# unlikeghost/DeepLearning-MPI

Measured on AMD Instinct MI355X. Metric: images/sec (whole node) ResNet-50 DDP bs=256/GPU, higher is better.
Workload: dtype bf16; 1 GPU; model=resnet50, global_batch=256, image=224, in_channels=3, per_gpu_batch=256, parallelism=dp1, backend=single, device=cuda, optimizer=SGD(momentum=0.9, wd=1e-5), hipgraph=False

## Files before the change

deeplearning_mpi_amd/csrc/binding/conv_fwd.cpp:

```cpp
#include <algorithm>
#include <cstdio>
#include <map>
#include <vector>

#include "common.h"

namespace dlmpi_ext {

using dlmpi::ConvArgs;
using dlmpi::ConvPhase;
using dlmpi::FinArgs;
using dlmpi::Stream1x1Args;
using dlmpi::make_fastdiv;

void apply_halo(ConvArgs& a, int N, int bm) {
  ConvPhase& p = a.ph[0];
  int th = 8, tw = 16, tiles_h = 1, tiles_w = 1;
  halo_geom(p.P, p.Q, bm, th, tw, tiles_h, tiles_w);
  a.halo = 1;
  a.th = th;
  a.tw = tw;
  a.tiles_h = tiles_h;
  a.tiles_w = tiles_w;
  a.fd_tw = make_fastdiv((uint32_t)tw);
// ... 282 lines not shown
      const bool c8 = pl.path == FwdPath::c8;
      check((c8 ? dlmpi_conv3x3_c8 : dlmpi_conv4x4_c16)(a.x, ldx, xoff, N, H, W, a.w, a.bias, a.y, ldy, yoff, a.stats,
                                                        pl.G, cur_stream()),
            c8 ? "conv2d_fwd (8-channel 3x3)" : "conv2d_fwd (stem 4x4 x 16 channels)");
      (c8 ? g_ran.c8 : g_ran.c16) = 1;
      break;
    }
    case FwdPath::head:
      check(dlmpi_head1x1(a.x, ldx, xoff, (int64_t)N * H * W, C, a.w, a.ldw, a.bias, a.y, ldy, yoff, a.kvalid,
                          o.y_f32 ? 1 : 0, nullptr, nullptr, cur_stream()),
            "conv2d_fwd (1x1 head)");
      g_ran.head = 1;
      return 0;
    case FwdPath::stream3x3: {
      dlmpi::Conv3StreamArgs c = conv3_args(x, N, H, W, ldx, xoff, w, 0, a.y, ldy, yoff, pl.th, pl.tw, pl.G);
      c.bias = a.bias;
      c.stats = a.stats;
      check(dlmpi_conv3x3_stream(&c, a.stats ? 0 : 1, cur_stream()), "conv2d_fwd (stream 3x3)");
      g_ran.conv3 = 1;
      break;
    }
    case FwdPath::stream1x1: {
      Stream1x1Args sa = fill_stream1x1(x, ldx, xoff, w, y, ldy, yoff, s.M(), C, K, a.bias, H, W, P, Q, pl.sbm,
                                        pl.sbn, pl.G);
      sa.stats = a.stats;
      sa.s2 = stride == 2 ? 1 : 0;
      check(dlmpi_conv1x1_stream(&sa, pl.sbm, pl.sbn, cur_stream()), "conv2d_fwd (stream 1x1)");
      g_ran.stream = 1;
      break;
    }
    case FwdPath::apply1x1:
      a.ntiles = ceil_div(K, bn);
      single_phase(a, P, Q, R, S, pad, bm);
      check(dlmpi_conv1x1_apply(&a, bm, cur_stream()), "conv2d_fwd (fused apply 1x1)");
      break;
    case FwdPath::pipe:
    case FwdPath::halo:
    case FwdPath::igemm:
      a.ntiles = ceil_div(K, bn);
      single_phase(a, P, Q, R, S, pad, bm);
      if (pl.path == FwdPath::halo) apply_halo(a, N, bm);
      g_ran.halo = pl.path == FwdPath::halo ? 1 : 0;
      if (!pl.pipe && (fin != nullptr || !a.stats) && s.free_tiles() && autotune(a, 0, bm, bn)) rows = a.ph[0].mtiles;
      if (fin != nullptr) need_rows(rows);
      if (g_sw.splitk > 0) a.splitk_req = g_sw.splitk;
      check(dlmpi_conv_igemm_ex(&a, bm, bn, pl.pipe, cur_stream()), "conv2d_fwd");
      break;
  }
  if (fin != nullptr) run_fin_after(*stats, rows, K, fin);
  return rows;
}

int conv2d_fwd_pro(const at::Tensor& x, int N, int H, int W, int C, int ldx, int xoff, const at::Tensor& w, int K, int R,
               int S, int stride, int pad, at::Tensor y, int ldy, int yoff, const c10::optional<at::Tensor>& bias,
               const c10::optional<at::Tensor>& res, int ldres, int resoff, const c10::optional<at::Tensor>& scale,
               const c10::optional<at::Tensor>& shift, bool relu, const c10::optional<at::Tensor>& stats, int bm_req,
               int kvalid, int bn_req, int pro, const c10::optional<at::Tensor>& pk0,
               const c10::optional<at::Tensor>& pk1, const c10::optional<at::Tensor>& pz, int ldpz, int pzoff) {
  return conv2d_fwd_impl(x, N, H, W, C, ldx, xoff, w, K, R, S, stride, pad, y, ldy, yoff, bias, res, ldres, resoff,
                         scale, shift, relu, stats, bm_req, kvalid, bn_req, pro, pk0, pk1, pz, ldpz, pzoff, nullptr);
}

int conv2d_fwd(const at::Tensor& x, int N, int H, int W, int C, int ldx, int xoff, const at::Tensor& w, int K, int R,
               int S, int stride, int pad, at::Tensor y, int ldy, int yoff, const c10::optional<at::Tensor>& bias,
               const c10::optional<at::Tensor>& res, int ldres, int resoff, const c10::optional<at::Tensor>& scale,
               const c10::optional<at::Tensor>& shift, bool relu, const c10::optional<at::Tensor>& stats, int bm_req,
               int kvalid, int bn_req) {
// ... 190 lines not shown
  check(dlmpi_conv_igemm(&a, t.bm, t.bn, cur_stream()), "convT2x2_fwd");
}

void register_conv_fwd(pybind11::module& m) {
  m.def("conv2d_fwd", &conv2d_fwd);
  m.def("conv2d_fwd_pro", &conv2d_fwd_pro);
  m.def("conv2d_fwd_bn", &conv2d_fwd_bn);
  m.def("conv2d_fwd_bn_apply", &conv2d_fwd_bn_apply);
  m.def("conv2d_fwd_mtiles", &conv2d_fwd_mtiles);
  m.def("conv2d_fwd_mtiles_pro", &conv2d_fwd_mtiles_pro);
  m.def("conv2d_fwd_plan", &conv2d_fwd_plan);
  m.def("conv_tune_tiles", [](int f32, int C, int K) {
    std::vector<std::pair<int, int>> v;
    for (const TuneCand& c : tune_candidates(f32, C, K, 0)) v.emplace_back(c.bm, c.bn);
    return v;
  });
  m.def("conv2d_fwd_bnbwd", &conv2d_fwd_bnbwd);
  m.def("convT2x2_fwd", &convT2x2_fwd);
  m.def("conv1x1_head_affine", &conv1x1_head_affine);
  m.def("conv3_pro_ok", &conv3_pro_ok);
  m.def("conv3x3_fwd_bn_apply", &conv3x3_fwd_bn_apply);
  m.def("clear_conv_plans", []() { g_conv_plans.clear(); });
  m.def("set_conv_stream", [](int mode) { dlmpi_set_conv_stream(mode); });
  m.def("set_conv3_stream", [](int mode) { dlmpi_set_conv3_stream(mode); });
  m.def("set_halo_pipe", [](int on) { dlmpi_set_halo_pipe(on); });
  m.def("set_dgs_blocks", [](int n) { dlmpi_set_dgs_blocks(n); });
  m.def("dgs_blocks", []() { return dlmpi_dgs_blocks(); });
  def_int(m, "set_conv_autotune", nullptr, &g_sw.autotune);
  def_int(m, "set_conv_halo", nullptr, &g_sw.halo);
  def_int(m, "set_halo_first", nullptr, &g_sw.halo_first);
  def_int(m, "set_conv_splitk", nullptr, &g_sw.splitk);
  def_int(m, "set_conv_pipe", nullptr, &g_sw.pipe);
  def_int(m, "set_conv_apply", nullptr, &g_sw.apply);
  def_int(m, "set_head1x1", "head1x1_on", &g_sw.head);
  def_int(m, "set_conv_c8", nullptr, &g_sw.c8);
  def_int(m, "set_conv_c16", nullptr, &g_sw.c16);
  def_int(m, "set_conv3_pro", nullptr, &g_sw.c3pro);
  def_int(m, "set_convT_stream", nullptr, &g_sw.convT_stream);
  def_int(m, nullptr, "conv_stream_last", &g_ran.stream);
  def_int(m, nullptr, "conv3_stream_last", &g_ran.conv3);
  def_int(m, nullptr, "conv_halo_last", &g_ran.halo);
  def_int(m, nullptr, "conv_c8_last", &g_ran.c8);
  def_int(m, nullptr, "conv_c16_last", &g_ran.c16);
  def_int(m, nullptr, "head1x1_last", &g_ran.head);
  def_int(m, nullptr, "convT_stream_last", &g_ran.convT_stream);
}

}
```

deeplearning_mpi_amd/csrc/binding/conv_plan.h:

```cpp
#pragma once
#include <cstdint>
#include <vector>

#include "../kernels/dlmpi_kernels.h"

namespace dlmpi_ext {

static inline int ceil_div(int64_t a, int64_t b) { return (int)((a + b - 1) / b); }

struct Switches {
  int pipe = -1;
  int pipe_dgrad = -1;
  int apply = -1;
  int halo = -1;
  int halo_first = 1;
  int splitk = 0;
  int autotune = -1;
  int head = 1;
  int c8 = 1;
  int c16 = 1;
  int c3pro = 1;
  int convT_stream = 1;
  int wgrad3 = -1;
  int wgrad3_blocks = 0;
  int wgrad_blocks = 0;
};
struct LastRan {
  int halo = 0;
  int stream = 0;
  int dgrad_stream = 0;
  int conv3 = 0;
  int head = 0;
  int c8 = 0;
  int c16 = 0;
  int convT_stream = 0;
  int wgrad3 = 0;
  int head_dgrad = 0;
};
extern Switches g_sw;
extern LastRan g_ran;
bool conv_autotune_on();

struct ConvShape {
  int N, H, W, C, K, R, S, stride, pad;
  int pro, f32;
  int bm_req, bn_req;
// ... 62 lines not shown
```

deeplearning_mpi_amd/csrc/kernels/conv_igemm.hip:

```cpp
#include <cstdlib>
#include <type_traits>

#include "common.h"

namespace dlmpi {

typedef __attribute__((address_space(3))) void lds_void;

__device__ __forceinline__ void glds16(const void* g, char* lds_wave_base) {
  __builtin_amdgcn_global_load_lds(g, (lds_void*)lds_wave_base, 16, 0, 0);
}

template <int BM, int BN, int NT, int WM>
struct EpiSmem {
  static constexpr int NP0 = BM < 128 ? 1 : (BM / 64 < WM / 16 ? BM / 64 : WM / 16);
  static constexpr int NP = (WM / 16) % NP0 == 0 ? NP0 : WM / 16;
  static constexpr int CS_LD = BN + 4;
  static constexpr int EPI = (BM / NP) * CS_LD * 4;
  static constexpr int RED = (NT / (BN / 8)) * 3 * BN * 4;
  static constexpr int bytes = EPI > RED ? EPI : RED;
};

template <int NT, int NF>
__device__ __forceinline__ bool splitk_combine(const ConvArgs& a, f32x4* acc, char* smem, int tid, int mt, int nt) {
  const int S = a.splitk;
  const int64_t tile = (int64_t)blockIdx.z * gridDim.x + (int64_t)mt * a.ntiles + nt;
  f32x4* slab = reinterpret_cast<f32x4*>(a.sk_slab) + (tile * S + blockIdx.y) * NF * NT + tid;
#pragma unroll
  for (int i = 0; i < NF; ++i) slab[(int64_t)i * NT] = acc[i];
  asm volatile("s_waitcnt vmcnt(0)" ::: "memory");
  __syncthreads();
  int* flag = reinterpret_cast<int*>(smem);
  if (tid == 0) {
    __builtin_amdgcn_fence(__ATOMIC_RELEASE, "agent");
    asm volatile("s_waitcnt vmcnt(0)" ::: "memory");
    flag[0] = __hip_atomic_fetch_add(a.sk_tk + tile, 1, __ATOMIC_RELAXED, __HIP_MEMORY_SCOPE_AGENT) == S - 1;
  }
  __syncthreads();
  if (!flag[0]) return false;
  if (tid == 0) {
    __builtin_amdgcn_fence(__ATOMIC_ACQUIRE, "agent");
    asm volatile("s_waitcnt vmcnt(0)" ::: "memory");
    __hip_atomic_store(a.sk_tk + tile, 0, __ATOMIC_RELAXED, __HIP_MEMORY_SCOPE_AGENT);
  }
  __syncthreads();
  const f32x4* base = reinterpret_cast<const f32x4*>(a.sk_slab) + tile * S * NF * NT + tid;
#pragma unroll
  for (int i = 0; i < NF; ++i) acc[i] = f32x4{0.f, 0.f, 0.f, 0.f};
  for (int sp = 0; sp < S; ++sp)
#pragma unroll
    for (int i = 0; i < NF; ++i) acc[i] += base[((int64_t)sp * NF + i) * NT];
  __syncthreads();
  return true;
}

template <int BM, int BN, int NT, int WGM, int WGN, typename T, bool HALO>
__device__ __forceinline__ void conv_epilogue(const ConvArgs& a, const ConvPhase& ph,
                                              f32x4 (&acc)[BM / WGM / 16][BN / WGN / 16], char* smem, int tid,
                                              int m0, int n0, int mt, int hn, int hh0, int hw0) {
  constexpr int WM = BM / WGM, WN = BN / WGN;
  constexpr int TM = WM / 16, TN = WN / 16;
  constexpr int NP = EpiSmem<BM, BN, NT, WM>::NP;
  constexpr int CS_LD = EpiSmem<BM, BN, NT, WM>::CS_LD;
  static_assert(WM % (16 * NP) == 0 || NP == 1, "epilogue pass must split every wave's rows evenly");
  const int lane = tid & 63;
  const int wid = __builtin_amdgcn_readfirstlane(tid >> 6);
  const int wm = wid / WGN, wn = wid % WGN;
  const int fr = lane & 15, fg = lane >> 4;
  const int PQ = ph.P * ph.Q;
  const int M = a.Nimg * PQ;
  float* Cs = reinterpret_cast<float*>(smem);

  constexpr int CG = BN / 8;
  constexpr int RG = NT / CG;
  const int cg = tid % CG, rg = tid / CG;
  const int c0 = n0 + cg * 8;
  const bool cvalid = c0 < a.Kout;
  float bias[8];
#pragma unroll
  for (int e = 0; e < 8; ++e) bias[e] = 0.f;
  if (cvalid && a.bias) {
#pragma unroll
    for (int e = 0; e < 8; ++e) bias[e] = a.bias[c0 + e];
  }
  float s1[8], s2[8], s3[8];
#pragma unroll
  for (int e = 0; e < 8; ++e) { s1[e] = 0.f; s2[e] = 0.f; s3[e] = 0.f; }
  const bool bwd = a.mask != nullptr || a.mscale != nullptr || a.mbits != nullptr;

  constexpr int HM = WM / NP, HT = TM / NP;
#pragma unroll
  for (int h = 0; h < NP; ++h) {
  if (h) __syncthreads();
#pragma unroll
  for (int mi = 0; mi < HT; ++mi)
#pragma unroll
    for (int ni = 0; ni < TN; ++ni)
#pragma unroll
      for (int r = 0; r < 4; ++r)
        Cs[(wm * HM + mi * 16 + fg * 4 + r) * CS_LD + wn * WN + ni * 16 + fr] = acc[h * HT + mi][ni][r];
  __syncthreads();
  constexpr int EPI_UNROLL = BM >= 256 ? 1 : 2;
#pragma unroll EPI_UNROLL
  for (int rr = rg; rr < BM / NP; rr += RG) {
    const int r = (rr / HM) * WM + h * HM + (rr % HM);
    const int m = m0 + r;
    int64_t pix;
    if constexpr (HALO) {
      const int pr = (int)fdiv((uint32_t)r, a.fd_tw), pc = r - pr * a.tw;
      const int oh = hh0 + pr, ow = hw0 + pc;
      if (r >= a.th * a.tw || oh >= ph.P || ow >= ph.Q || !cvalid) continue;
      pix = ((int64_t)hn * a.OH + oh * a.so + ph.oh0) * a.OW + ow * a.so + ph.ow0;
    } else {
      if (m >= M || !cvalid) continue;
    }
    float v[8];
    const f32x4 v0 = *reinterpret_cast<const f32x4*>(Cs + rr * CS_LD + cg * 8);
    const f32x4 v1 = *reinterpret_cast<const f32x4*>(Cs + rr * CS_LD + cg * 8 + 4);
#pragma unroll
    for (int e = 0; e < 4; ++e) { v[e] = v0[e] + bias[e]; v[e + 4] = v1[e] + bias[e + 4]; }
    if (a.stats && !bwd) {
#pragma unroll
      for (int e = 0; e < 8; ++e) {
        const float rv = stored<T>(v[e]);
        s1[e] += rv;
        s2[e] += rv * rv;
      }
    }
    if (a.scale) {
#pragma unroll
      for (int e = 0; e < 8; ++e) v[e] = v[e] * a.scale[c0 + e] + a.shift[c0 + e];
    }
    if constexpr (!HALO) {
      const uint32_t n_img = fdiv((uint32_t)m, ph.fdPQ);
      const uint32_t rem = (uint32_t)m - n_img * PQ;
      const uint32_t p = fdiv(rem, ph.fdQ);
      const uint32_t q = rem - p * ph.Q;
      pix = ((int64_t)n_img * a.OH + (int)p * a.so + ph.oh0) * a.OW + (int)q * a.so + ph.ow0;
    }
    if (a.res) {
      float rr8[8];
      load8(static_cast<const T*>(a.res) + pix * a.ldres + a.resoff + c0, rr8);
#pragma unroll
      for (int e = 0; e < 8; ++e) v[e] += rr8[e];
    }
    if (a.relu) {
#pragma unroll
      for (int e = 0; e < 8; ++e) v[e] = fmaxf(v[e], 0.f);
    }
    if (bwd) {
      float zz[8];
      if (a.z) load8(static_cast<const T*>(a.z) + pix * a.ldz + a.zoff + c0, zz);
      if (a.mbits) {
        const uint32_t b = a.mbits[pix * (a.Kout >> 3) + (c0 >> 3)];
#pragma unroll
        for (int e = 0; e < 8; ++e) v[e] = (b >> e) & 1u ? v[e] : 0.f;
      } else if (a.mask) {
        float yy[8];
        load8(static_cast<const T*>(a.mask) + pix * a.ldmask + a.maskoff + c0, yy);
#pragma unroll
        for (int e = 0; e < 8; ++e) v[e] = yy[e] > 0.f ? v[e] : 0.f;
      } else {
#pragma unroll
        for (int e = 0; e < 8; ++e) v[e] = zz[e] * a.mscale[c0 + e] + a.mshift[c0 + e] > 0.f ? v[e] : 0.f;
      }
      if (a.stats) {
#pragma unroll
        for (int e = 0; e < 8; ++e) {
          const float rv = stored<T>(v[e]);
          s1[e] += rv;
          s2[e] += rv * zz[e];
        }
        if (a.z2) {
          load8(static_cast<const T*>(a.z2) + pix * a.ldz2 + a.z2off + c0, zz);
#pragma unroll
          for (int e = 0; e < 8; ++e) s3[e] += stored<T>(v[e]) * zz[e];
        }
      }
    }
    if (a.vec_store) {
      if (a.out_f32) {
        float* yp = reinterpret_cast<float*>(a.y) + pix * a.ldy + a.yoff + c0;
        *reinterpret_cast<f32x4*>(yp) = f32x4{v[0], v[1], v[2], v[3]};
        *reinterpret_cast<f32x4*>(yp + 4) = f32x4{v[4], v[5], v[6], v[7]};
      } else {
        uint16_t* yp = reinterpret_cast<uint16_t*>(a.y) + pix * a.ldy + a.yoff + c0;
        *reinterpret_cast<u32x4*>(yp) = pack8(v);
      }
    } else {
#pragma unroll
      for (int e = 0; e < 8; ++e) {
        if (c0 + e >= a.kvalid) break;
        if (a.out_f32) reinterpret_cast<float*>(a.y)[pix * a.ldy + a.yoff + c0 + e] = v[e];
        else reinterpret_cast<uint16_t*>(a.y)[pix * a.ldy + a.yoff + c0 + e] = f2bf(v[e]);
      }
    }
  }
  }

  if (a.stats) {
    __syncthreads();
    float* red = reinterpret_cast<float*>(smem);
    const int ns = a.nstat;
#pragma unroll
    for (int e = 0; e < 8; ++e) {
      red[(rg * 3 + 0) * BN + cg * 8 + e] = s1[e];
      red[(rg * 3 + 1) * BN + cg * 8 + e] = s2[e];
      red[(rg * 3 + 2) * BN + cg * 8 + e] = s3[e];
    }
    __syncthreads();
    if (tid < BN && n0 + tid < a.Kout) {
      float t1 = 0.f, t2 = 0.f, t3 = 0.f;
      for (int g = 0; g < RG; ++g) {
// ... 703 lines not shown
      bf16x8 af[TM], bfr[TN];
#pragma unroll
      for (int ni = 0; ni < TN; ++ni)
        bfr[ni] = *reinterpret_cast<const bf16x8*>(smem + b_row0 + sl * B_BYTES + ni * 16 * 128 + ((ch ^ sw) << 4));
#pragma unroll
      for (int mi = 0; mi < TM; ++mi)
        af[mi] = *reinterpret_cast<const bf16x8*>(smem + (kk ? (a_addr[mi] ^ 64) : a_addr[mi]));
      if (kk == 0 && more && !chunk_end) {
        issue_b(sl ^ 1);
        asm volatile("" ::: "memory");
      }
#pragma unroll
      for (int mi = 0; mi < TM; ++mi)
#pragma unroll
        for (int ni = 0; ni < TN; ++ni)
          acc[mi][ni] = __builtin_amdgcn_mfma_f32_16x16x32_bf16(af[mi], bfr[ni], acc[mi][ni], 0, 0, 0);
    }
    if (chunk_end) {
      asm volatile("s_waitcnt lgkmcnt(0)" ::: "memory");
      __builtin_amdgcn_s_barrier();
      asm volatile("" ::: "memory");
      issue_halo();
      issue_b(sl ^ 1);
    }
  };
  for (int ks = 0; ks < nk; ks += 2) {
    step(ks, std::integral_constant<int, 0>{});
    if (ks + 1 < nk) step(ks + 1, std::integral_constant<int, 1>{});
  }
  __syncthreads();
  conv_epilogue<BM, BN, NT, WGM, WGN, uint16_t, true>(a, ph, acc, smem, tid, m0, n0, mt, hn, hh0, hw0);
}

template <int BM, int BN, int WGM, int WGN>
__global__ __launch_bounds__(512) __attribute__((amdgpu_waves_per_eu(BN <= 128 ? 4 : 2, 8)))
void conv1x1_apply_kernel(const ConvArgs a) {
  constexpr int NT = 512;
  static_assert(WGM * WGN == 8, "8 waves");
  constexpr int WM = BM / WGM, WN = BN / WGN, TM = WM / 16, TN = WN / 16;
  constexpr int A_BYTES = BM * 128, B_BYTES = BN * 128, SB = A_BYTES + B_BYTES;
  constexpr int MAXC = 4 * BN;
  constexpr int PRM_BYTES = 4 * MAXC * 4;
  constexpr int EPI_NEED = EpiSmem<BM, BN, NT, WM>::bytes;
  constexpr int SMEM = 2 * SB + PRM_BYTES > EPI_NEED ? 2 * SB + PRM_BYTES : EPI_NEED;
  constexpr int RP = NT / 8;
  constexpr int AL = BM / RP, BL = BN / RP;
  static_assert(AL >= 1 && BL >= 1, "tile shape");
  __shared__ __attribute__((aligned(16))) char smem[SMEM];

  const int tid = threadIdx.x, lane = tid & 63;
  const int wid = __builtin_amdgcn_readfirstlane(tid >> 6);
  const int wm = wid / WGN, wn = wid % WGN;
  const int lrow = tid >> 3, jc = tid & 7;
  const ConvPhase& ph = a.ph[0];
  const int M = a.Nimg * ph.P * ph.Q;
  const uint32_t mt = xcd_remap(blockIdx.x, (uint32_t)ph.mtiles);
  const int m0 = (int)mt * BM;
  const int C = a.C, nk = C / 64;
  const bool rbn = a.prscale != nullptr;

  float* prm = reinterpret_cast<float*>(smem + 2 * SB);
  for (int i = tid; i < C; i += NT) {
    prm[i] = a.pscale[i];
    prm[MAXC + i] = a.pshift[i];
    if (rbn) {
      prm[2 * MAXC + i] = a.prscale[i];
      prm[3 * MAXC + i] = a.prshift[i];
    }
  }

  const uint16_t* xb = static_cast<const uint16_t*>(a.x);
  const uint16_t* rb = static_cast<const uint16_t*>(a.pz);
  uint32_t zo[AL], ro[AL], yo[AL], bo[AL];
  uint32_t okm = 0;
#pragma unroll
  for (int i = 0; i < AL; ++i) {
    const int m = m0 + lrow + RP * i;
    if (m < M) okm |= 1u << i;
    const uint32_t mm = m < M ? (uint32_t)m : 0u;
    zo[i] = mm * (uint32_t)a.ldx + (uint32_t)a.xoff + 8 * jc;
    ro[i] = mm * (uint32_t)a.ldpz + (uint32_t)a.pzoff + 8 * jc;
    yo[i] = mm * (uint32_t)a.ldpy + (uint32_t)a.pyoff + 8 * jc;
    bo[i] = mm * (uint32_t)(C >> 3) + jc;
  }
  const uint16_t* wb = static_cast<const uint16_t*>(a.w) + (int64_t)lrow * a.ldw + 8 * jc;
  const int64_t wstep = (int64_t)RP * a.ldw;

  u32x4 zv[AL], rv[AL], wv[BL];
  auto load = [&](int k) {
    const int c = 64 * k;
#pragma unroll
    for (int i = 0; i < AL; ++i) {
      zv[i] = *reinterpret_cast<const u32x4*>(xb + zo[i] + c);
      rv[i] = *reinterpret_cast<const u32x4*>(rb + ro[i] + c);
    }
#pragma unroll
    for (int i = 0; i < BL; ++i) wv[i] = *reinterpret_cast<const u32x4*>(wb + i * wstep + c);
  };
  auto commit = [&](int k, int buf) {
    char* As = smem + buf * SB;
    char* Bs = As + A_BYTES;
    const int cc = 64 * k + 8 * jc;
    const f32x4 s0 = *reinterpret_cast<const f32x4*>(prm + cc), s1 = *reinterpret_cast<const f32x4*>(prm + cc + 4);
    const f32x4 h0 = *reinterpret_cast<const f32x4*>(prm + MAXC + cc);
    const f32x4 h1 = *reinterpret_cast<const f32x4*>(prm + MAXC + cc + 4);
#pragma unroll
    for (int i = 0; i < AL; ++i) {
      const int r = lrow + RP * i;
      u32x4 pk = u32x4{0u, 0u, 0u, 0u};
      if ((okm >> i) & 1) {
        float v[8], q[8];
        unpack8(zv[i], v);
        unpack8(rv[i], q);
#pragma unroll
        for (int e = 0; e < 4; ++e) {
          v[e] = __builtin_fmaf(v[e], s0[e], h0[e]);
          v[e + 4] = __builtin_fmaf(v[e + 4], s1[e], h1[e]);
        }
        if (rbn) {
          const f32x4 a0 = *reinterpret_cast<const f32x4*>(prm + 2 * MAXC + cc);
          const f32x4 a1 = *reinterpret_cast<const f32x4*>(prm + 2 * MAXC + cc + 4);
          const f32x4 b0 = *reinterpret_cast<const f32x4*>(prm + 3 * MAXC + cc);
          const f32x4 b1 = *reinterpret_cast<const f32x4*>(prm + 3 * MAXC + cc + 4);
#pragma unroll
          for (int e = 0; e < 4; ++e) {
            q[e] = __builtin_fmaf(q[e], a0[e], b0[e]);
            q[e + 4] = __builtin_fmaf(q[e + 4], a1[e], b1[e]);
          }
        }
#pragma unroll
        for (int e = 0; e < 8; ++e) v[e] = fmaxf(v[e] + q[e], 0.f);
        pk = pack8(v);
        *reinterpret_cast<u32x4*>(a.py + yo[i] + 64 * k) = pk;
        uint32_t b = 0;
#pragma unroll
        for (int t = 0; t < 4; ++t) {
          b |= (uint32_t)((pk[t] & 0xffffu) != 0u && !(pk[t] & 0x8000u)) << (2 * t);
          b |= (uint32_t)((pk[t] >> 16) != 0u && !(pk[t] & 0x80000000u)) << (2 * t + 1);
        }
        a.pmbits[bo[i] + 8 * k] = (uint8_t)b;
      }
      *reinterpret_cast<u32x4*>(As + r * 128 + ((jc ^ (r & 7)) << 4)) = pk;
    }
#pragma unroll
    for (int i = 0; i < BL; ++i) {
      const int r = lrow + RP * i;
      *reinterpret_cast<u32x4*>(Bs + r * 128 + ((jc ^ (r & 7)) << 4)) = wv[i];
    }
  };

  f32x4 acc[TM][TN];
#pragma unroll
  for (int mi = 0; mi < TM; ++mi)
#pragma unroll
    for (int ni = 0; ni < TN; ++ni) acc[mi][ni] = f32x4{0.f, 0.f, 0.f, 0.f};
  const int fr = lane & 15, fg = lane >> 4;

  load(0);
  __syncthreads();
  commit(0, 0);
  __syncthreads();
  for (int k = 0; k < nk; ++k) {
    if (k + 1 < nk) load(k + 1);
    const char* As = smem + (k & 1) * SB;
    const char* Bs = As + A_BYTES;
#pragma unroll
    for (int kk = 0; kk < 2; ++kk) {
      bf16x8 af[TM], bfr[TN];
      const int ch = kk * 4 + fg;
#pragma unroll
      for (int mi = 0; mi < TM; ++mi) {
        const int r = wm * WM + mi * 16 + fr;
        af[mi] = *reinterpret_cast<const bf16x8*>(As + r * 128 + ((ch ^ (r & 7)) << 4));
      }
#pragma unroll
      for (int ni = 0; ni < TN; ++ni) {
        const int r = wn * WN + ni * 16 + fr;
        bfr[ni] = *reinterpret_cast<const bf16x8*>(Bs + r * 128 + ((ch ^ (r & 7)) << 4));
      }
#pragma unroll
      for (int mi = 0; mi < TM; ++mi)
#pragma unroll
        for (int ni = 0; ni < TN; ++ni)
          acc[mi][ni] = __builtin_amdgcn_mfma_f32_16x16x32_bf16(af[mi], bfr[ni], acc[mi][ni], 0, 0, 0);
    }
    if (k + 1 < nk) commit(k + 1, (k + 1) & 1);
    __syncthreads();
  }
  conv_epilogue<BM, BN, NT, WGM, WGN, uint16_t, false>(a, ph, acc, smem, tid, m0, 0, (int)mt, 0, 0, 0);
}

}

using namespace dlmpi;

template <int BM, int BN>
static hipError_t launch_tile(const ConvArgs* a, dim3 grid, hipStream_t s) {
  if (a->pro == 3) {
    if constexpr (BM == 128 && BN == 64) hipLaunchKernelGGL((conv_igemm_kernel<BM, BN, false, 2, 3>), grid, dim3(256), 0, s, *a);
    else return hipErrorInvalidValue;
  } else if (a->C < 64) hipLaunchKernelGGL((conv_igemm_kernel<BM, BN, true, 2>), grid, dim3(256), 0, s, *a);
  else hipLaunchKernelGGL((conv_igemm_kernel<BM, BN, false, 2>), grid, dim3(256), 0, s, *a);
  return hipSuccess;
}

static int splitk_plan(int tiles, int nk) {
  if (tiles >= 256 || nk < 8) return 1;
  int S = (256 + tiles - 1) / tiles;
  S = S < nk / 4 ? S : nk / 4;
  S = S < 8 ? S : 8;
  return S < 2 ? 1 : S;
}

static hipError_t launch_f32(const ConvArgs* a, int bm, int bn, dim3 grid, hipStream_t s) {
  if (a->pro != 0) return hipErrorInvalidValue;
  const bool small = a->C < 32 || a->C % 32 != 0;
#define LAUNCH_F32(BM_, BN_)                                                                                   \
  do {                                                                                                       \
    if (small) hipLaunchKernelGGL((conv_igemm_kernel<BM_, BN_, true, 2, 0, float>), grid, dim3(256), 0, s, *a); \
    else hipLaunchKernelGGL((conv_igemm_kernel<BM_, BN_, false, 2, 0, float>), grid, dim3(256), 0, s, *a);     \
  } while (0)
  if (bm == 128 && bn == 128) LAUNCH_F32(128, 128);
  else if (bm == 128 && bn == 64) LAUNCH_F32(128, 64);
  else if (bm == 64 && bn == 128) LAUNCH_F32(64, 128);
  else if (bm == 64 && bn == 64) LAUNCH_F32(64, 64);
  else return hipErrorInvalidValue;
#undef LAUNCH_F32
  return hipGetLastError();
}

static hipError_t launch_pipe(const ConvArgs* a, int bm, int bn, int var, dim3 grid, hipStream_t s) {
  if (a->f32 || a->pro != 0 || a->C % 64 != 0 || a->C > kPipeMaxC || a->halo || grid.y != 1) return hipErrorInvalidValue;
  if (var != (bm == 128 ? 4 : 2)) return hipErrorInvalidValue;
  if (bm == 256 && bn == 256) hipLaunchKernelGGL((conv_pipe_kernel<256, 256, 2, 4, 2, 2>), grid, dim3(512), 0, s, *a);
  else if (bm == 224 && bn == 256) hipLaunchKernelGGL((conv_pipe_kernel<224, 256, 2, 4, 2, 2>), grid, dim3(512), 0, s, *a);
  else if (bm == 256 && bn == 128) hipLaunchKernelGGL((conv_pipe_kernel<256, 128, 4, 2, 3, 2>), grid, dim3(512), 0, s, *a);
  else if (bm == 128 && bn == 256) hipLaunchKernelGGL((conv_pipe_kernel<128, 256, 2, 4, 3, 4>), grid, dim3(512), 0, s, *a);
  else if (bm == 512 && bn == 64) hipLaunchKernelGGL((conv_pipe_kernel<512, 64, 8, 1, 2, 2>), grid, dim3(512), 0, s, *a);
  else return hipErrorInvalidValue;
  return hipGetLastError();
}

extern "C" int dlmpi_conv1x1_apply_ok(int C, int K) {
  return C % 64 == 0 && C <= 4 * K && (K == 64 || K == 128 || K == 256);
}

extern "C" hipError_t dlmpi_conv1x1_apply(const ConvArgs* a, int bm, hipStream_t s) {
  if (a->pro != 3 || a->f32 || a->halo || a->nphase != 1 || a->ntiles != 1 || !a->vec_store || a->res ||
      a->scale || a->relu || a->mask || a->mscale || a->mbits || a->z || a->splitk_req > 1 ||
      !dlmpi_conv1x1_apply_ok(a->C, a->Kout) || a->ph[0].Tr != 1 || a->ph[0].Ts != 1 || a->sa != 1 ||
      a->ph[0].mtiles != (a->Nimg * a->ph[0].P * a->ph[0].Q + bm - 1) / bm || a->ldw != a->C ||
      (int64_t)a->Nimg * a->H * a->W * (a->ldx > a->ldpz ? (a->ldx > a->ldpy ? a->ldx : a->ldpy)
                                                          : (a->ldpz > a->ldpy ? a->ldpz : a->ldpy)) >= (1ll << 31))
    return hipErrorInvalidValue;
  const dim3 grid((unsigned)a->ph[0].mtiles);
  if (grid.x == 0) return hipSuccess;
  if (bm == 128 && a->Kout == 64) hipLaunchKernelGGL((conv1x1_apply_kernel<128, 64, 8, 1>), grid, dim3(512), 0, s, *a);
  else if (bm == 128 && a->Kout == 128) hipLaunchKernelGGL((conv1x1_apply_kernel<128, 128, 4, 2>), grid, dim3(512), 0, s, *a);
  else if (bm == 128 && a->Kout == 256) hipLaunchKernelGGL((conv1x1_apply_kernel<128, 256, 2, 4>), grid, dim3(512), 0, s, *a);
  else return hipErrorInvalidValue;
  return hipGetLastError();
}

static int g_halo_pipe = 1;
extern "C" void dlmpi_set_halo_pipe(int on) { g_halo_pipe = on; }

extern "C" hipError_t dlmpi_conv_igemm_ex(const ConvArgs* a_in, int bm, int bn, int pipe, hipStream_t s) {
  int maxt = 0, tiles = 0, maxk = 0;
  for (int i = 0; i < a_in->nphase; ++i) {
    maxt = a_in->ph[i].mtiles > maxt ? a_in->ph[i].mtiles : maxt;
    tiles += a_in->ph[i].mtiles * a_in->ntiles;
    maxk = a_in->ph[i].ksteps > maxk ? a_in->ph[i].ksteps : maxk;
  }
  ConvArgs ab = *a_in;
  const ConvArgs* a = &ab;
  ab.splitk = 1;
  if (pipe) {
    const dim3 grid((unsigned)(maxt * a->ntiles), 1, (unsigned)a->nphase);
    if (grid.x == 0) return hipSuccess;
    return launch_pipe(a, bm, bn, pipe - 1, grid, s);
  }
  int S = a_in->splitk_req > 0 ? a_in->splitk_req : splitk_plan(tiles, maxk);
  if (S > maxk) S = maxk > 0 ? maxk : 1;
  if (S > 1) {
    const int ntile_ids = maxt * a_in->ntiles * a_in->nphase;
    float* slab = dlmpi_splitk_slab(s, (size_t)ntile_ids * S * bm * bn);
    int* tk = dlmpi_splitk_tickets(s, ntile_ids);
    if (slab && tk) {
      ab.splitk = S;
      ab.sk_slab = slab;
      ab.sk_tk = tk;
    }
  }
  dim3 grid((unsigned)(maxt * a->ntiles), (unsigned)ab.splitk, (unsigned)a->nphase);
// ... 32 lines not shown
```

deeplearning_mpi_amd/csrc/kernels/dlmpi_kernels.h:

```cpp
#pragma once
#include <hip/hip_runtime_api.h>
#include <stdint.h>

namespace dlmpi {

struct FastDiv {
  uint32_t d, mul, shr;
};
inline FastDiv make_fastdiv(uint32_t d) {
  FastDiv f;
  f.d = d;
  uint32_t l = 0;
  while ((1ull << l) < d) ++l;
  f.mul = (uint32_t)((((1ull << 32) * ((1ull << l) - d)) / d) + 1);
  f.shr = l;
  return f;
}

struct FinArgs {
  int mode;
  double count;
  const float* gamma;
  const float* beta;
  float* running_mean;
// ... 162 lines not shown
  const float* ws;
  float* ws2;
  float* out;
  int64_t total;
  int splits, G, Ko_real, T, Cpad, Creal;
  int block1;
  int block2;
};
constexpr int kWgradBatch = 16;
struct WgradReduceBatch {
  int n;
  WgradReduceEntry e[kWgradBatch];
};

struct Wgrad3Args {
  const void* dy;
  int ldy, dyoff, Ko;
  const void* x;
  int ldx, xoff, C;
  int H, W;
  int tiles_h, tiles_w, ntiles_pix, tiles_per_split;
  int mtiles, ntiles, splits;
  float* ws;
};

}

extern "C" {
void dlmpi_set_wgrad_fast(int on);
void dlmpi_set_halo_pipe(int on);
hipError_t dlmpi_conv_igemm(const dlmpi::ConvArgs* a, int bm, int bn, hipStream_t s);
hipError_t dlmpi_conv_igemm_ex(const dlmpi::ConvArgs* a, int bm, int bn, int pipe, hipStream_t s);
int dlmpi_conv1x1_apply_ok(int C, int K);
hipError_t dlmpi_conv1x1_apply(const dlmpi::ConvArgs* a, int bm, hipStream_t s);
hipError_t dlmpi_conv_wgrad(const dlmpi::WgradArgs* a, int bm, int bn, hipStream_t s);
int dlmpi_wgrad_pro_ok(int direct, int pro_a, int pro_b);
hipError_t dlmpi_wgrad_reduce(const float* ws, int splits, int Ko, int T, int Cpad, int Creal,
                              int Ko_real, float* out, float* ws2, int ws2_floats, hipStream_t s);
int dlmpi_wgrad_reduce_groups(int splits, int64_t total);
hipError_t dlmpi_wgrad_reduce_batch(dlmpi::WgradReduceBatch* b, hipStream_t s);
int dlmpi_wgrad3_plan(int Ko, int C, int* kt, int* ct);
hipError_t dlmpi_wgrad3x3(const dlmpi::Wgrad3Args* a, int kt, int ct, hipStream_t s);
int dlmpi_head1x1_ok(int C, int kv);
int dlmpi_conv3x3_c8_blocks(int64_t pixels);
int dlmpi_conv4x4_c16_blocks(int64_t pixels);
hipError_t dlmpi_conv4x4_c16(const void* x, int ldx, int xoff, int N, int U, int V, const void* w, const float* bias,
                             void* y, int ldy, int yoff, float* stats, int G, hipStream_t s);
hipError_t dlmpi_conv3x3_c8(const void* x, int ldx, int xoff, int N, int H, int W, const void* w, const float* bias,
                            void* y, int ldy, int yoff, float* stats, int G, hipStream_t s);
hipError_t dlmpi_head1x1(const void* x, int ldx, int xoff, int64_t M, int C, const void* w, int ldw,
                         const float* bias, void* y, int ldy, int yoff, int kv, int y_f32, const float* psc,
                         const float* psh, hipStream_t s);
int dlmpi_conv3_stream_plan(int N, int H, int W, int C, int K, int blocks, int* th, int* tw, int* G);
hipError_t dlmpi_conv3x3_stream(const dlmpi::Conv3StreamArgs* a, int mode, hipStream_t s);
void dlmpi_set_conv3_stream(int mode);

hipError_t dlmpi_bn_finalize(const float* partial, int ntiles, int C, double count, const float* gamma,
                             const float* beta, float* running_mean, float* running_var, float momentum,
                             float eps, float* scale, float* shift, float* save_mean, float* save_invstd,
                             double* ws, hipStream_t s);
int dlmpi_colsum_ws_doubles(int T, int C);
hipError_t dlmpi_set_aux_stream(hipStream_t s, int role);
hipError_t dlmpi_bn_stats(const void* x, int64_t M, int C, int ldx, int xoff, float* partial, int nblk, int f32,
                          hipStream_t s);
hipError_t dlmpi_bn_apply(const void* x, int ldx, int xoff, int64_t M, int C, const float* scale, const float* shift,
                          const void* res, int ldres, int resoff, int relu, void* y, int ldy, int yoff, uint8_t* mbits,
                          int f32, hipStream_t s);
// ... 122 lines not shown
```

Before: 13760 images/sec.

## Make fused 1x1 apply conv persistent with LDS-resident weights and plain epilogue

The fused BN-apply 1x1 conv kernel becomes a persistent grid-stride kernel whose grid is capped at resident occupancy. For K=64 it can keep the full weight matrix resident in LDS across tiles, and it prefetches the next tile's activations during the epilogue. A PLAIN epilogue specialization drops the residual, scale and relu branches, which this path never uses. This is meant to cut per-block weight reloads and launch/tail overhead, at the cost of extra LDS use, lower waves per EU for the resident-weight variant, and more complex control flow.

```diff
diff --git a/deeplearning_mpi_amd/csrc/binding/conv_fwd.cpp b/deeplearning_mpi_amd/csrc/binding/conv_fwd.cpp
--- a/deeplearning_mpi_amd/csrc/binding/conv_fwd.cpp
+++ b/deeplearning_mpi_amd/csrc/binding/conv_fwd.cpp
@@ -338,7 +338,7 @@
     case FwdPath::apply1x1:
       a.ntiles = ceil_div(K, bn);
       single_phase(a, P, Q, R, S, pad, bm);
-      check(dlmpi_conv1x1_apply(&a, bm, cur_stream()), "conv2d_fwd (fused apply 1x1)");
+      check(dlmpi_conv1x1_apply(&a, bm, g_sw.apply_blocks, cur_stream()), "conv2d_fwd (fused apply 1x1)");
       break;
     case FwdPath::pipe:
     case FwdPath::halo:
@@ -595,6 +595,8 @@
   def_int(m, "set_conv_splitk", nullptr, &g_sw.splitk);
   def_int(m, "set_conv_pipe", nullptr, &g_sw.pipe);
   def_int(m, "set_conv_apply", nullptr, &g_sw.apply);
+  def_int(m, "set_conv_apply_blocks", nullptr, &g_sw.apply_blocks);
+  m.def("set_conv_apply_resw", [](int mode) { dlmpi_set_apply_resw(mode); });
   def_int(m, "set_head1x1", "head1x1_on", &g_sw.head);
   def_int(m, "set_conv_c8", nullptr, &g_sw.c8);
   def_int(m, "set_conv_c16", nullptr, &g_sw.c16);
diff --git a/deeplearning_mpi_amd/csrc/binding/conv_plan.h b/deeplearning_mpi_amd/csrc/binding/conv_plan.h
--- a/deeplearning_mpi_amd/csrc/binding/conv_plan.h
+++ b/deeplearning_mpi_amd/csrc/binding/conv_plan.h
@@ -12,6 +12,7 @@
   int pipe = -1;
   int pipe_dgrad = -1;
   int apply = -1;
+  int apply_blocks = 0;
   int halo = -1;
   int halo_first = 1;
   int splitk = 0;
diff --git a/deeplearning_mpi_amd/csrc/kernels/conv_igemm.hip b/deeplearning_mpi_amd/csrc/kernels/conv_igemm.hip
--- a/deeplearning_mpi_amd/csrc/kernels/conv_igemm.hip
+++ b/deeplearning_mpi_amd/csrc/kernels/conv_igemm.hip
@@ -54,7 +54,7 @@
   return true;
 }
 
-template <int BM, int BN, int NT, int WGM, int WGN, typename T, bool HALO>
+template <int BM, int BN, int NT, int WGM, int WGN, typename T, bool HALO, bool PLAIN = false>
 __device__ __forceinline__ void conv_epilogue(const ConvArgs& a, const ConvPhase& ph,
                                               f32x4 (&acc)[BM / WGM / 16][BN / WGN / 16], char* smem, int tid,
                                               int m0, int n0, int mt, int hn, int hh0, int hw0) {
@@ -86,7 +86,7 @@
   float s1[8], s2[8], s3[8];
 #pragma unroll
   for (int e = 0; e < 8; ++e) { s1[e] = 0.f; s2[e] = 0.f; s3[e] = 0.f; }
-  const bool bwd = a.mask != nullptr || a.mscale != nullptr || a.mbits != nullptr;
+  const bool bwd = !PLAIN && (a.mask != nullptr || a.mscale != nullptr || a.mbits != nullptr);
 
   constexpr int HM = WM / NP, HT = TM / NP;
 #pragma unroll
@@ -100,7 +100,7 @@
       for (int r = 0; r < 4; ++r)
         Cs[(wm * HM + mi * 16 + fg * 4 + r) * CS_LD + wn * WN + ni * 16 + fr] = acc[h * HT + mi][ni][r];
   __syncthreads();
-  constexpr int EPI_UNROLL = BM >= 256 ? 1 : 2;
+  constexpr int EPI_UNROLL = BM >= 256 || PLAIN ? 1 : 2;
 #pragma unroll EPI_UNROLL
   for (int rr = rg; rr < BM / NP; rr += RG) {
     const int r = (rr / HM) * WM + h * HM + (rr % HM);
@@ -127,7 +127,7 @@
         s2[e] += rv * rv;
       }
     }
-    if (a.scale) {
+    if (!PLAIN && a.scale) {
 #pragma unroll
       for (int e = 0; e < 8; ++e) v[e] = v[e] * a.scale[c0 + e] + a.shift[c0 + e];
     }
@@ -138,13 +138,13 @@
       const uint32_t q = rem - p * ph.Q;
       pix = ((int64_t)n_img * a.OH + (int)p * a.so + ph.oh0) * a.OW + (int)q * a.so + ph.ow0;
     }
-    if (a.res) {
+    if (!PLAIN && a.res) {
       float rr8[8];
       load8(static_cast<const T*>(a.res) + pix * a.ldres + a.resoff + c0, rr8);
 #pragma unroll
       for (int e = 0; e < 8; ++e) v[e] += rr8[e];
     }
-    if (a.relu) {
+    if (!PLAIN && a.relu) {
 #pragma unroll
       for (int e = 0; e < 8; ++e) v[e] = fmaxf(v[e], 0.f);
     }
@@ -178,7 +178,7 @@
         }
       }
     }
-    if (a.vec_store) {
+    if (PLAIN || a.vec_store) {
       if (a.out_f32) {
         float* yp = reinterpret_cast<float*>(a.y) + pix * a.ldy + a.yoff + c0;
         *reinterpret_cast<f32x4*>(yp) = f32x4{v[0], v[1], v[2], v[3]};
@@ -948,21 +948,39 @@
   conv_epilogue<BM, BN, NT, WGM, WGN, uint16_t, true>(a, ph, acc, smem, tid, m0, n0, mt, hn, hh0, hw0);
 }
 
-template <int BM, int BN, int WGM, int WGN>
-__global__ __launch_bounds__(512) __attribute__((amdgpu_waves_per_eu(BN <= 128 ? 4 : 2, 8)))
+template <int BM, int BN, int WGM, bool RESW>
+struct ApplySmem {
+  static constexpr int NT = 512;
+  static constexpr int A_BYTES = BM * 128, B_BYTES = BN * 128;
+  static constexpr int SB = A_BYTES + (RESW ? 0 : B_BYTES);
+  static constexpr int EPI_NEED = EpiSmem<BM, BN, NT, BM / WGM>::bytes;
+  static constexpr int WORK = 2 * SB > EPI_NEED ? 2 * SB : EPI_NEED;
+  static constexpr int LDS_BUDGET = 160 * 1024;
+  static constexpr int res_maxc() {
+    int c = 4 * BN;
+    while (c > 0 && WORK + BN * c * 2 + 4 * c * 4 > LDS_BUDGET) c -= 64;
+    return c;
+  }
+  static constexpr int MAXC = RESW ? res_maxc() : 4 * BN;
+  static constexpr int W_BYTES = RESW ? BN * MAXC * 2 : 0;
+  static constexpr int PRM_BYTES = 4 * MAXC * 4;
+  static constexpr int bytes = WORK + W_BYTES + PRM_BYTES;
+  static_assert(MAXC >= 64 && bytes <= LDS_BUDGET, "LDS budget");
+};
+
+template <int BM, int BN, int WGM, int WGN, bool RESW>
+__global__ __launch_bounds__(512) __attribute__((amdgpu_waves_per_eu(BN <= 128 && !RESW ? 4 : 2, 8)))
 void conv1x1_apply_kernel(const ConvArgs a) {
-  constexpr int NT = 512;
+  using L = ApplySmem<BM, BN, WGM, RESW>;
+  constexpr int NT = L::NT;
   static_assert(WGM * WGN == 8, "8 waves");
   constexpr int WM = BM / WGM, WN = BN / WGN, TM = WM / 16, TN = WN / 16;
-  constexpr int A_BYTES = BM * 128, B_BYTES = BN * 128, SB = A_BYTES + B_BYTES;
-  constexpr int MAXC = 4 * BN;
-  constexpr int PRM_BYTES = 4 * MAXC * 4;
-  constexpr int EPI_NEED = EpiSmem<BM, BN, NT, WM>::bytes;
-  constexpr int SMEM = 2 * SB + PRM_BYTES > EPI_NEED ? 2 * SB + PRM_BYTES : EPI_NEED;
+  constexpr int A_BYTES = L::A_BYTES, B_BYTES = L::B_BYTES, SB = L::SB;
+  constexpr int MAXC = L::MAXC;
   constexpr int RP = NT / 8;
   constexpr int AL = BM / RP, BL = BN / RP;
   static_assert(AL >= 1 && BL >= 1, "tile shape");
-  __shared__ __attribute__((aligned(16))) char smem[SMEM];
+  __shared__ __attribute__((aligned(16))) char smem[L::bytes];
 
   const int tid = threadIdx.x, lane = tid & 63;
   const int wid = __builtin_amdgcn_readfirstlane(tid >> 6);
@@ -970,12 +988,13 @@
   const int lrow = tid >> 3, jc = tid & 7;
   const ConvPhase& ph = a.ph[0];
   const int M = a.Nimg * ph.P * ph.Q;
-  const uint32_t mt = xcd_remap(blockIdx.x, (uint32_t)ph.mtiles);
-  const int m0 = (int)mt * BM;
+  const int G = (int)gridDim.x, mtiles = ph.mtiles;
+  int mt = (int)xcd_remap(blockIdx.x, gridDim.x);
   const int C = a.C, nk = C / 64;
   const bool rbn = a.prscale != nullptr;
 
-  float* prm = reinterpret_cast<float*>(smem + 2 * SB);
+  char* Wres = smem + L::WORK;
+  float* prm = reinterpret_cast<float*>(smem + L::WORK + L::W_BYTES);
   for (int i = tid; i < C; i += NT) {
     prm[i] = a.pscale[i];
     prm[MAXC + i] = a.pshift[i];
@@ -984,34 +1003,55 @@
       prm[3 * MAXC + i] = a.prshift[i];
     }
   }
-
-  const uint16_t* xb = static_cast<const uint16_t*>(a.x);
-  const uint16_t* rb = static_cast<const uint16_t*>(a.pz);
-  uint32_t zo[AL], ro[AL], yo[AL], bo[AL];
+  const char* wb = static_cast<const char*>(a.w);
+  const uint32_t wo = 2u * (uint32_t)(lrow * a.ldw + 8 * jc), wstep = 2u * (uint32_t)(RP * a.ldw);
+  if constexpr (RESW) {
+    for (int k = 0; k < nk; ++k)
+#pragma unroll
+      for (int i = 0; i < BL; ++i) {
+        const int r = lrow + RP * i;
+        *reinterpret_cast<u32x4*>(Wres + k * B_BYTES + r * 128 + ((jc ^ (r & 7)) << 4)) =
+            *reinterpret_cast<const u32x4*>(wb + (wo + i * wstep + 128u * k));
+      }
+  }
+
+  const char* xb = static_cast<const char*>(a.x);
+  const char* rb = static_cast<const char*>(a.pz);
+  char* yb = reinterpret_cast<char*>(a.py);
+  uint32_t mrow[AL];
   uint32_t okm = 0;
-#pragma unroll
-  for (int i = 0; i < AL; ++i) {
-    const int m = m0 + lrow + RP * i;
-    if (m < M) okm |= 1u << i;
-    const uint32_t mm = m < M ? (uint32_t)m : 0u;
-    zo[i] = mm * (uint32_t)a.ldx + (uint32_t)a.xoff + 8 * jc;
-    ro[i] = mm * (uint32_t)a.ldpz + (uint32_t)a.pzoff + 8 * jc;
-    yo[i] = mm * (uint32_t)a.ldpy + (uint32_t)a.pyoff + 8 * jc;
-    bo[i] = mm * (uint32_t)(C >> 3) + jc;
-  }
-  const uint16_t* wb = static_cast<const uint16_t*>(a.w) + (int64_t)lrow * a.ldw + 8 * jc;
-  const int64_t wstep = (int64_t)RP * a.ldw;
-
-  u32x4 zv[AL], rv[AL], wv[BL];
+  auto rows = [&](int m0) {
+    okm = 0;
+#pragma unroll
+    for (int i = 0; i < AL; ++i) {
+      const int m = m0 + lrow + RP * i;
+      if (m < M) okm |= 1u << i;
+      mrow[i] = m < M ? (uint32_t)m : 0u;
+    }
+  };
+  auto row_off = [&](int i, int ld, int off) {
+    uint32_t mm = mrow[i];
+    asm volatile("" : "+v"(mm));
+    return 2u * (mm * (uint32_t)ld + (uint32_t)off + 8 * jc);
+  };
+
+  u32x4 zv[AL], rv[AL], wv[RESW ? 1 : BL];
+  auto load_a = [&](int k) {
+#pragma unroll
+    for (int i = 0; i < AL; ++i) {
+      zv[i] = *reinterpret_cast<const u32x4*>(xb + (row_off(i, a.ldx, a.xoff) + 128u * k));
+      rv[i] = *reinterpret_cast<const u32x4*>(rb + (row_off(i, a.ldpz, a.pzoff) + 128u * k));
+    }
+  };
+  auto load_w = [&](int k) {
+    if constexpr (!RESW) {
+#pragma unroll
+      for (int i = 0; i < BL; ++i) wv[i] = *reinterpret_cast<const u32x4*>(wb + (wo + i * wstep + 128u * k));
+    }
+  };
   auto load = [&](int k) {
-    const int c = 64 * k;
-#pragma unroll
-    for (int i = 0; i < AL; ++i) {
-      zv[i] = *reinterpret_cast<const u32x4*>(xb + zo[i] + c);
-      rv[i] = *reinterpret_cast<const u32x4*>(rb + ro[i] + c);
-    }
-#pragma unroll
-    for (int i = 0; i < BL; ++i) wv[i] = *reinterpret_cast<const u32x4*>(wb + i * wstep + c);
+    load_a(k);
+    load_w(k);
   };
   auto commit = [&](int k, int buf) {
     char* As = smem + buf * SB;
@@ -1047,63 +1087,84 @@
 #pragma unroll
         for (int e = 0; e < 8; ++e) v[e] = fmaxf(v[e] + q[e], 0.f);
         pk = pack8(v);
-        *reinterpret_cast<u32x4*>(a.py + yo[i] + 64 * k) = pk;
+        *reinterpret_cast<u32x4*>(yb + (row_off(i, a.ldpy, a.pyoff) + 128u * k)) = pk;
         uint32_t b = 0;
 #pragma unroll
         for (int t = 0; t < 4; ++t) {
           b |= (uint32_t)((pk[t] & 0xffffu) != 0u && !(pk[t] & 0x8000u)) << (2 * t);
           b |= (uint32_t)((pk[t] >> 16) != 0u && !(pk[t] & 0x80000000u)) << (2 * t + 1);
         }
-        a.pmbits[bo[i] + 8 * k] = (uint8_t)b;
+        uint32_t mm = mrow[i];
+        asm volatile("" : "+v"(mm));
+        a.pmbits[mm * (uint32_t)(C >> 3) + jc + 8u * k] = (uint8_t)b;
       }
       *reinterpret_cast<u32x4*>(As + r * 128 + ((jc ^ (r & 7)) << 4)) = pk;
     }
-#pragma unroll
-    for (int i = 0; i < BL; ++i) {
-      const int r = lrow + RP * i;
-      *reinterpret_cast<u32x4*>(Bs + r * 128 + ((jc ^ (r & 7)) << 4)) = wv[i];
-    }
-  };
-
-  f32x4 acc[TM][TN];
-#pragma unroll
-  for (int mi = 0; mi < TM; ++mi)
-#pragma unroll
-    for (int ni = 0; ni < TN; ++ni) acc[mi][ni] = f32x4{0.f, 0.f, 0.f, 0.f};
+    if constexpr (!RESW) {
+#pragma unroll
+      for (int i = 0; i < BL; ++i) {
+        const int r = lrow + RP * i;
+        *reinterpret_cast<u32x4*>(Bs + r * 128 + ((jc ^ (r & 7)) << 4)) = wv[i];
+      }
+    }
+  };
+
   const int fr = lane & 15, fg = lane >> 4;
-
+  rows(mt * BM);
   load(0);
   __syncthreads();
-  commit(0, 0);
-  __syncthreads();
-  for (int k = 0; k < nk; ++k) {
-    if (k + 1 < nk) load(k + 1);
-    const char* As = smem + (k & 1) * SB;
-    const char* Bs = As + A_BYTES;
-#pragma unroll
-    for (int kk = 0; kk < 2; ++kk) {
-      bf16x8 af[TM], bfr[TN];
-      const int ch = kk * 4 + fg;
-#pragma unroll
-      for (int mi = 0; mi < TM; ++mi) {
-        const int r = wm * WM + mi * 16 + fr;
-        af[mi] = *reinterpret_cast<const bf16x8*>(As + r * 128 + ((ch ^ (r & 7)) << 4));
-      }
-#pragma unroll
-      for (int ni = 0; ni < TN; ++ni) {
-        const int r = wn * WN + ni * 16 + fr;
-        bfr[ni] = *reinterpret_cast<const bf16x8*>(Bs + r * 128 + ((ch ^ (r & 7)) << 4));
-      }
-#pragma unroll
-      for (int mi = 0; mi < TM; ++mi)
-#pragma unroll
-        for (int ni = 0; ni < TN; ++ni)
-          acc[mi][ni] = __builtin_amdgcn_mfma_f32_16x16x32_bf16(af[mi], bfr[ni], acc[mi][ni], 0, 0, 0);
-    }
-    if (k + 1 < nk) commit(k + 1, (k + 1) & 1);
+  while (true) {
+    const int m0 = mt * BM;
+    commit(0, 0);
     __syncthreads();
-  }
-  conv_epilogue<BM, BN, NT, WGM, WGN, uint16_t, false>(a, ph, acc, smem, tid, m0, 0, (int)mt, 0, 0, 0);
+    f32x4 acc[TM][TN];
+#pragma unroll
+    for (int mi = 0; mi < TM; ++mi)
+#pragma unroll
+      for (int ni = 0; ni < TN; ++ni) acc[mi][ni] = f32x4{0.f, 0.f, 0.f, 0.f};
+    for (int k = 0; k < nk; ++k) {
+      if (k + 1 < nk) load(k + 1);
+      const char* As = smem + (k & 1) * SB;
+      const char* Bs = RESW ? Wres + k * B_BYTES : As + A_BYTES;
+#pragma unroll
+      for (int kk = 0; kk < 2; ++kk) {
+        bf16x8 af[TM], bfr[TN];
+        const int ch = kk * 4 + fg;
+#pragma unroll
+        for (int mi = 0; mi < TM; ++mi) {
+          const int r = wm * WM + mi * 16 + fr;
+          af[mi] = *reinterpret_cast<const bf16x8*>(As + r * 128 + ((ch ^ (r & 7)) << 4));
+        }
+#pragma unroll
+        for (int ni = 0; ni < TN; ++ni) {
+          const int r = wn * WN + ni * 16 + fr;
+          bfr[ni] = *reinterpret_cast<const bf16x8*>(Bs + r * 128 + ((ch ^ (r & 7)) << 4));
+        }
+#pragma unroll
+        for (int mi = 0; mi < TM; ++mi)
+#pragma unroll
+          for (int ni = 0; ni < TN; ++ni)
+            acc[mi][ni] = __builtin_amdgcn_mfma_f32_16x16x32_bf16(af[mi], bfr[ni], acc[mi][ni], 0, 0, 0);
+      }
+      if (k + 1 < nk) commit(k + 1, (k + 1) & 1);
+      __syncthreads();
+    }
+    const int nmt = mt + G;
+    if (nmt < mtiles) {
+      rows(nmt * BM);
+      load_a(0);
+    }
+    int tid_e = tid;
+    asm volatile("" : "+v"(tid_e));
+    conv_epilogue<BM, BN, NT, WGM, WGN, uint16_t, false, true>(a, ph, acc, smem, tid_e, m0, 0, mt, 0, 0, 0);
+    if (nmt >= mtiles) break;
+    mt = nmt;
+    int m0n = mt * BM;
+    asm volatile("" : "+s"(m0n));
+    rows(m0n);
+    load_w(0);
+    __syncthreads();
+  }
 }
 
 }
@@ -1161,7 +1222,32 @@
   return C % 64 == 0 && C <= 4 * K && (K == 64 || K == 128 || K == 256);
 }
 
-extern "C" hipError_t dlmpi_conv1x1_apply(const ConvArgs* a, int bm, hipStream_t s) {
+static int g_apply_resw = -1;
+extern "C" void dlmpi_set_apply_resw(int mode) { g_apply_resw = mode; }
+
+template <int BN, int WGM, int WGN, bool RESW>
+static hipError_t launch_apply(const ConvArgs* a, bool persistent, int cap, hipStream_t s) {
+  static int resident = 0;
+  if (resident == 0) {
+    int dev = 0, cus = 0, per_cu = 0;
+    hipError_t e = hipGetDevice(&dev);
+    if (e == hipSuccess) e = hipDeviceGetAttribute(&cus, hipDeviceAttributeMultiprocessorCount, dev);
+    if (e == hipSuccess)
+      e = hipOccupancyMaxActiveBlocksPerMultiprocessor(&per_cu, conv1x1_apply_kernel<128, BN, WGM, WGN, RESW>, 512, 0);
+    if (e != hipSuccess) return e;
+    if (cus < 1 || per_cu < 1) return hipErrorInvalidValue;
+    resident = cus * per_cu;
+  }
+  int g = a->ph[0].mtiles;
+  if (persistent && resident < g) g = resident;
+  if (cap > 0 && cap < g) g = cap;
+  hipLaunchKernelGGL((conv1x1_apply_kernel<128, BN, WGM, WGN, RESW>), dim3((unsigned)g), dim3(512), 0, s, *a);
+  return hipGetLastError();
+}
+
+static bool apply_persistent_rule(int C, int K) { return K == 64 || (K == 256 && C <= 512); }
+
+extern "C" hipError_t dlmpi_conv1x1_apply(const ConvArgs* a, int bm, int blocks_cap, hipStream_t s) {
   if (a->pro != 3 || a->f32 || a->halo || a->nphase != 1 || a->ntiles != 1 || !a->vec_store || a->res ||
       a->scale || a->relu || a->mask || a->mscale || a->mbits || a->z || a->splitk_req > 1 ||
       !dlmpi_conv1x1_apply_ok(a->C, a->Kout) || a->ph[0].Tr != 1 || a->ph[0].Ts != 1 || a->sa != 1 ||
@@ -1169,13 +1255,17 @@
       (int64_t)a->Nimg * a->H * a->W * (a->ldx > a->ldpz ? (a->ldx > a->ldpy ? a->ldx : a->ldpy)
                                                           : (a->ldpz > a->ldpy ? a->ldpz : a->ldpy)) >= (1ll << 31))
     return hipErrorInvalidValue;
-  const dim3 grid((unsigned)a->ph[0].mtiles);
-  if (grid.x == 0) return hipSuccess;
-  if (bm == 128 && a->Kout == 64) hipLaunchKernelGGL((conv1x1_apply_kernel<128, 64, 8, 1>), grid, dim3(512), 0, s, *a);
-  else if (bm == 128 && a->Kout == 128) hipLaunchKernelGGL((conv1x1_apply_kernel<128, 128, 4, 2>), grid, dim3(512), 0, s, *a);
-  else if (bm == 128 && a->Kout == 256) hipLaunchKernelGGL((conv1x1_apply_kernel<128, 256, 2, 4>), grid, dim3(512), 0, s, *a);
-  else return hipErrorInvalidValue;
-  return hipGetLastError();
+  if (bm != 128) return hipErrorInvalidValue;
+  if (a->ph[0].mtiles == 0) return hipSuccess;
+  const int K = a->Kout, C = a->C;
+  const bool pers = blocks_cap >= 0 && apply_persistent_rule(C, K);
+  if (K == 64) {
+    if (pers && g_apply_resw != 0 && C <= ApplySmem<128, 64, 8, true>::MAXC)
+      return launch_apply<64, 8, 1, true>(a, pers, blocks_cap, s);
+    return launch_apply<64, 8, 1, false>(a, pers, blocks_cap, s);
+  }
+  if (K == 128) return launch_apply<128, 4, 2, false>(a, pers, blocks_cap, s);
+  return launch_apply<256, 2, 4, false>(a, pers, blocks_cap, s);
 }
 
 static int g_halo_pipe = 1;
diff --git a/deeplearning_mpi_amd/csrc/kernels/dlmpi_kernels.h b/deeplearning_mpi_amd/csrc/kernels/dlmpi_kernels.h
--- a/deeplearning_mpi_amd/csrc/kernels/dlmpi_kernels.h
+++ b/deeplearning_mpi_amd/csrc/kernels/dlmpi_kernels.h
@@ -218,7 +218,8 @@
 hipError_t dlmpi_conv_igemm(const dlmpi::ConvArgs* a, int bm, int bn, hipStream_t s);
 hipError_t dlmpi_conv_igemm_ex(const dlmpi::ConvArgs* a, int bm, int bn, int pipe, hipStream_t s);
 int dlmpi_conv1x1_apply_ok(int C, int K);
-hipError_t dlmpi_conv1x1_apply(const dlmpi::ConvArgs* a, int bm, hipStream_t s);
+hipError_t dlmpi_conv1x1_apply(const dlmpi::ConvArgs* a, int bm, int blocks_cap, hipStream_t s);
+void dlmpi_set_apply_resw(int mode);
 hipError_t dlmpi_conv_wgrad(const dlmpi::WgradArgs* a, int bm, int bn, hipStream_t s);
 int dlmpi_wgrad_pro_ok(int direct, int pro_a, int pro_b);
 hipError_t dlmpi_wgrad_reduce(const float* ws, int splits, int Ko, int T, int Cpad, int Creal,
```

Result: no change. 13800 images/sec, median of 6 (+0.3%).
